# addtt/ladder-vae-pytorch

Measured on NVIDIA B200. Metric: train images/s (CIFAR10 15-layer LVAE), higher is better.
Workload: dtype bf16

## Files before the change

### ladder-vae-pytorch_b200/csrc/wgrad_tcgen05.cu

```cuda
#include "common.cuh"
#include <cuda.h>
#include <string.h>

namespace {

constexpr int WG_THREADS_TC = 192;
constexpr int WG_TILE = 128;
constexpr int WG_BLK_BYTES = WG_TILE * 64 * 2;
constexpr int WG_MAX_PAIRS = 5;
constexpr int WG_PAIR_SLOTS = 4;
constexpr int WG_B_SLOTS = 2;
constexpr int WG_HALO_BYTES = 18 * 16 * 128;
constexpr int WG_HALO_STAGE_BYTES = WG_HALO_BYTES + WG_BLK_BYTES;
constexpr int WG_HALO_STAGES = 3;

struct WgParams {
  int M_total, H, W;
  int n_pairs;
  int n_bblk;
  int tmem_cols;
  int tiles_per_cta;
  int dy_c0;
  int halo, tiles_x, tiles_per_img;
  int in_stride;

  int8_t a_src[2 * WG_MAX_PAIRS], a_dx[2 * WG_MAX_PAIRS], a_dy[2 * WG_MAX_PAIRS];
};

__device__ __forceinline__ uint32_t smem_u32(const void* p) { return (uint32_t)__cvta_generic_to_shared(p); }
__device__ __forceinline__ void mbar_init(uint32_t bar, uint32_t count) {
  asm volatile("mbarrier.init.shared::cta.b64 [%0], %1;" ::"r"(bar), "r"(count));
}
__device__ __forceinline__ void mbar_expect_tx(uint32_t bar, uint32_t bytes) {
  asm volatile("mbarrier.arrive.expect_tx.shared::cta.b64 _, [%0], %1;" ::"r"(bar), "r"(bytes) : "memory");
}
__device__ __forceinline__ uint32_t mbar_try_wait(uint32_t bar, uint32_t parity) {
  uint32_t ok;
  asm volatile(
      "{\n\t.reg .pred p;\n\t"
      "mbarrier.try_wait.parity.shared::cta.b64 p, [%1], %2;\n\t"
      "selp.u32 %0, 1, 0, p;\n\t}"
      : "=r"(ok) : "r"(bar), "r"(parity) : "memory");
  return ok;
}
__device__ __forceinline__ void mbar_wait(uint32_t bar, uint32_t parity) {
  while (!mbar_try_wait(bar, parity)) {}
}
__device__ __forceinline__ void tma_load_4d(uint32_t dst, const CUtensorMap* tm, uint32_t bar, int c0, int c1, int c2, int c3) {
  asm volatile(
      "cp.async.bulk.tensor.4d.shared::cluster.global.mbarrier::complete_tx::bytes [%0], [%1, {%3, %4, %5, %6}], [%2];"
      ::"r"(dst), "l"(tm), "r"(bar), "r"(c0), "r"(c1), "r"(c2), "r"(c3) : "memory");
}
__device__ __forceinline__ uint64_t umma_desc_mn_sw128(uint32_t saddr, uint32_t lbo_bytes, uint32_t sbo_bytes = 1024) {
  uint64_t d = 0;
  d |= (uint64_t)((saddr & 0x3FFFF) >> 4);
  d |= (uint64_t)((lbo_bytes >> 4) & 0x3FFF) << 16;
  d |= (uint64_t)(sbo_bytes >> 4) << 32;
  d |= (uint64_t)1 << 46;
  d |= (uint64_t)2 << 61;
  return d;
}
__device__ __forceinline__ void umma_bf16(uint32_t d_tmem, uint64_t adesc, uint64_t bdesc, uint32_t idesc, uint32_t accumulate) {
  asm volatile(
      "{\n\t.reg .pred p;\n\t"
      "setp.ne.b32 p, %4, 0;\n\t"
      "tcgen05.mma.cta_group::1.kind::f16 [%0], %1, %2, %3, p;\n\t}"
      ::"r"(d_tmem), "l"(adesc), "l"(bdesc), "r"(idesc), "r"(accumulate) : "memory");
}
__device__ __forceinline__ uint32_t elect_one() {
  uint32_t pred = 0;
  asm volatile(
      "{\n\t.reg .pred p;\n\t"
      "elect.sync _|p, 0xffffffff;\n\t"
      "selp.u32 %0, 1, 0, p;\n\t}"
      : "=r"(pred));
  return pred;
}
__device__ __forceinline__ void umma_commit(uint32_t bar) {
  asm volatile("tcgen05.commit.cta_group::1.mbarrier::arrive::one.shared::cluster.b64 [%0];" ::"r"(bar) : "memory");
}
__device__ __forceinline__ void tc_fence_before() { asm volatile("tcgen05.fence::before_thread_sync;" ::: "memory"); }
__device__ __forceinline__ void tc_fence_after() { asm volatile("tcgen05.fence::after_thread_sync;" ::: "memory"); }
__device__ __forceinline__ void tmem_ld32(uint32_t taddr, uint32_t* r) {
  asm volatile(
      "tcgen05.ld.sync.aligned.32x32b.x32.b32 {%0,%1,%2,%3,%4,%5,%6,%7,%8,%9,%10,%11,%12,%13,%14,%15,"
      "%16,%17,%18,%19,%20,%21,%22,%23,%24,%25,%26,%27,%28,%29,%30,%31}, [%32];"
      : "=r"(r[0]), "=r"(r[1]), "=r"(r[2]), "=r"(r[3]), "=r"(r[4]), "=r"(r[5]), "=r"(r[6]), "=r"(r[7]), "=r"(r[8]),
        "=r"(r[9]), "=r"(r[10]), "=r"(r[11]), "=r"(r[12]), "=r"(r[13]), "=r"(r[14]), "=r"(r[15]), "=r"(r[16]),
        "=r"(r[17]), "=r"(r[18]), "=r"(r[19]), "=r"(r[20]), "=r"(r[21]), "=r"(r[22]), "=r"(r[23]), "=r"(r[24]),
        "=r"(r[25]), "=r"(r[26]), "=r"(r[27]), "=r"(r[28]), "=r"(r[29]), "=r"(r[30]), "=r"(r[31])
      : "r"(taddr));
  asm volatile("tcgen05.wait::ld.sync.aligned;" ::: "memory");
}

__global__ void __launch_bounds__(WG_THREADS_TC, 1)
wgrad_tc_kernel(const __grid_constant__ CUtensorMap tmX, const __grid_constant__ CUtensorMap tmX2,
                const __grid_constant__ CUtensorMap tmDY, const __grid_constant__ CUtensorMap tmGp, const WgParams p) {
  extern __shared__ uint8_t smem_raw[];
  uint8_t* smem = smem_raw + ((1024u - (smem_u32(smem_raw) & 1023u)) & 1023u);
  uint8_t* sPair = smem;
  uint8_t* sB = sPair + WG_PAIR_SLOTS * 2 * WG_BLK_BYTES;
  uint8_t* sOnes = p.halo ? smem + WG_HALO_STAGES * WG_HALO_STAGE_BYTES
                          : sB + WG_B_SLOTS * p.n_bblk * WG_BLK_BYTES;
  uint64_t* bars = (uint64_t*)(sOnes + WG_BLK_BYTES);
  uint32_t* tmem_slot = (uint32_t*)(bars + 16);
  const uint32_t bar0 = smem_u32(bars);
  auto BAR = [&](int i) { return bar0 + 8u * (uint32_t)i; };
  const int warp = threadIdx.x >> 5, lane = threadIdx.x & 31;
  const int n_tiles = p.halo ? (p.M_total / (p.H * p.W)) * p.tiles_per_img : (p.M_total + WG_TILE - 1) / WG_TILE;
  const int tile_beg = blockIdx.x * p.tiles_per_cta;
  const int tile_end = min(n_tiles, tile_beg + p.tiles_per_cta);
  const int N = 64 * p.n_bblk;

  if (threadIdx.x == 0) {
    for (int i = 0; i < 13; ++i) mbar_init(BAR(i), 1);
    asm volatile("fence.mbarrier_init.release.cluster;" ::: "memory");
  }
  for (int i = threadIdx.x; i < WG_BLK_BYTES / 4; i += WG_THREADS_TC) ((uint32_t*)sOnes)[i] = 0x3F803F80u;
  asm volatile("fence.proxy.async.shared::cta;" ::: "memory");
  if (warp == 1) {
    asm volatile("tcgen05.alloc.cta_group::1.sync.aligned.shared::cta.b32 [%0], %1;" ::"r"(smem_u32(tmem_slot)), "r"(p.tmem_cols) : "memory");
    asm volatile("tcgen05.relinquish_alloc_permit.cta_group::1.sync.aligned;" ::: "memory");
  }
  tc_fence_before();
  __syncthreads();
  tc_fence_after();
  const uint32_t tmem_base = *tmem_slot;
  pdl_wait();
  pdl_launch();

  if (warp == 0) {
    if (p.halo) {
      int st = 0;
      uint32_t ph = 0;
      for (int tile = tile_beg; tile < tile_end; ++tile) {
        const int n0 = tile / p.tiles_per_img;
        const int r = tile - n0 * p.tiles_per_img;
        const int ty = r / p.tiles_x, tx = r - ty * p.tiles_x;
        mbar_wait(BAR(4 + st), ph ^ 1);
        if (elect_one()) {
          uint8_t* stage = smem + st * WG_HALO_STAGE_BYTES;
          mbar_expect_tx(BAR(st), (uint32_t)WG_HALO_STAGE_BYTES);
          tma_load_4d(smem_u32(stage), &tmX, BAR(st), 0, tx * 8 - 1, ty * 16 - 1, n0);
          tma_load_4d(smem_u32(stage + WG_HALO_BYTES), &tmDY, BAR(st), p.dy_c0, tx * 8, ty * 16, n0);
        }
        __syncwarp();
        if (++st == WG_HALO_STAGES) { st = 0; ph ^= 1; }
      }
    } else {
      const int hw = p.H * p.W;
      int ps = 0, bs = 0;
      uint32_t pph = 0, bph = 0;
      for (int tile = tile_beg; tile < tile_end; ++tile) {
        int p0 = tile * WG_TILE;
        int n0 = p0 / hw;
        int rem = p0 - n0 * hw;
        int h0 = rem / p.W;
        int w0 = rem - h0 * p.W;
        mbar_wait(BAR(10 + bs), bph ^ 1);
        if (elect_one()) {
          mbar_expect_tx(BAR(8 + bs), (uint32_t)(p.n_bblk * WG_BLK_BYTES));
          for (int j = 0; j < p.n_bblk; ++j)
            tma_load_4d(smem_u32(sB + (bs * p.n_bblk + j) * WG_BLK_BYTES), &tmDY, BAR(8 + bs), p.dy_c0 + 64 * j, w0, h0, n0);
        }
        __syncwarp();
        if (++bs == WG_B_SLOTS) { bs = 0; bph ^= 1; }
        for (int pr = 0; pr < p.n_pairs; ++pr) {
          mbar_wait(BAR(4 + ps), pph ^ 1);
          if (elect_one()) {
            int nload = 0;
            for (int h = 0; h < 2; ++h) nload += p.a_src[2 * pr + h] < 2 ? 1 : 0;
            mbar_expect_tx(BAR(ps), (uint32_t)(nload * WG_BLK_BYTES));
            for (int h = 0; h < 2; ++h) {
              int src = p.a_src[2 * pr + h];
              if (src < 2)
                tma_load_4d(smem_u32(sPair + (ps * 2 + h) * WG_BLK_BYTES), src ? &tmX2 : &tmX, BAR(ps), 0,
                            w0 * p.in_stride + p.a_dx[2 * pr + h], h0 * p.in_stride + p.a_dy[2 * pr + h], n0);
            }
          }
          __syncwarp();
          if (++ps == WG_PAIR_SLOTS) { ps = 0; pph ^= 1; }
        }
      }
    }
  } else if (warp == 1) {
    {
      const uint32_t tmem_u = __shfl_sync(0xffffffffu, tmem_base, 0);
      const uint32_t idesc = (1u << 4) | (1u << 7) | (1u << 10) | (1u << 15) | (1u << 16) |
                             ((uint32_t)(N >> 3) << 17) | ((uint32_t)(128 >> 4) << 24);
      int ps = 0, bs = 0;
      uint32_t pph = 0, bph = 0;
      if (p.halo) {
        int st = 0;
        uint32_t ph = 0;
        const uint32_t ones = smem_u32(sOnes);
        for (int tile = tile_beg; tile < tile_end; ++tile) {
          mbar_wait(BAR(st), ph);
          tc_fence_after();
          const uint32_t h_addr = smem_u32(smem + st * WG_HALO_STAGE_BYTES);
          const uint32_t b_addr = h_addr + WG_HALO_BYTES;
          if (elect_one()) {
            for (int pr = 0; pr < p.n_pairs; ++pr) {
              const uint32_t a0 = h_addr + (uint32_t)(((1 + p.a_dy[2 * pr]) * 16 + (1 + p.a_dx[2 * pr])) * 128);
              const bool second_ones = p.a_src[2 * pr + 1] == 2;
              const uint32_t a1 = h_addr + (uint32_t)(((1 + p.a_dy[2 * pr + 1]) * 16 + (1 + p.a_dx[2 * pr + 1])) * 128);
              const uint32_t d_tmem = tmem_u + (uint32_t)(pr * N);
#pragma unroll
              for (int k = 0; k < WG_TILE / 16; ++k) {
                const uint32_t ak = a0 + k * 4096;
                const uint32_t lbo = second_ones ? ones - ak : a1 - a0;
                umma_bf16(d_tmem, umma_desc_mn_sw128(ak, lbo, 2048), umma_desc_mn_sw128(b_addr + k * 2048, WG_BLK_BYTES),
                          idesc, (uint32_t)((tile != tile_beg) || k != 0));
              }
            }
            umma_commit(BAR(4 + st));
          }
          __syncwarp();
          if (++st == WG_HALO_STAGES) { st = 0; ph ^= 1; }
        }
        if (elect_one()) umma_commit(BAR(12));
        __syncwarp();
      } else {
      for (int tile = tile_beg; tile < tile_end; ++tile) {
        mbar_wait(BAR(8 + bs), bph);
        tc_fence_after();
        const uint32_t b_addr = smem_u32(sB + bs * p.n_bblk * WG_BLK_BYTES);
        for (int pr = 0; pr < p.n_pairs; ++pr) {
          mbar_wait(BAR(ps), pph);
          tc_fence_after();
          const uint32_t a_addr = smem_u32(sPair + ps * 2 * WG_BLK_BYTES);
          const uint32_t a2 = p.a_src[2 * pr + 1] == 2 ? smem_u32(sOnes) : a_addr + WG_BLK_BYTES;
          const uint32_t lbo_a = a2 - a_addr;
          const uint32_t d_tmem = tmem_u + (uint32_t)(pr * N);
          if (elect_one()) {
#pragma unroll
            for (int k = 0; k < WG_TILE / 16; ++k) {
              umma_bf16(d_tmem, umma_desc_mn_sw128(a_addr + k * 2048, lbo_a), umma_desc_mn_sw128(b_addr + k * 2048, WG_BLK_BYTES),
                        idesc, (uint32_t)((tile != tile_beg) || k != 0));
            }
            umma_commit(BAR(4 + ps));
          }
          __syncwarp();
          if (++ps == WG_PAIR_SLOTS) { ps = 0; pph ^= 1; }
        }
        if (elect_one()) umma_commit(BAR(10 + bs));
        __syncwarp();
        if (++bs == WG_B_SLOTS) { bs = 0; bph ^= 1; }
      }
      if (elect_one()) umma_commit(BAR(12));
      __syncwarp();
      }
    }
  } else {
    const int quad = warp & 3;
    const int row = quad * 32 + lane;
    const bool leader = threadIdx.x == 64;
    mbar_wait(BAR(12), 0);
    tc_fence_after();
    if (tile_beg < tile_end) {
      int nbuf = 0;
      for (int pr = 0; pr < p.n_pairs; ++pr) {
        const uint32_t taddr = tmem_base + ((uint32_t)(quad * 32) << 16) + (uint32_t)(pr * N);
        for (int c0 = 0; c0 < N; c0 += 32, ++nbuf) {
          uint8_t* stg = smem + (nbuf & 1) * WG_BLK_BYTES;
          uint32_t r[32];
          tmem_ld32(taddr + (uint32_t)c0, r);
          if (leader) asm volatile("cp.async.bulk.wait_group.read 1;" ::: "memory");
          asm volatile("bar.sync 1, 128;" ::: "memory");
#pragma unroll
          for (int q = 0; q < 8; ++q)
            *reinterpret_cast<uint4*>(stg + row * 128 + ((q ^ (row & 7)) << 4)) = make_uint4(r[4 * q], r[4 * q + 1], r[4 * q + 2], r[4 * q + 3]);
          asm volatile("fence.proxy.async.shared::cta;" ::: "memory");
          asm volatile("bar.sync 1, 128;" ::: "memory");
          if (leader) {
            asm volatile("cp.reduce.async.bulk.tensor.2d.global.shared::cta.add.tile.bulk_group [%0, {%2, %3}], [%1];"
                         ::"l"(&tmGp), "r"(smem_u32(stg)), "r"(c0), "r"(pr * 128) : "memory");
            asm volatile("cp.async.bulk.commit_group;" ::: "memory");
          }
        }
      }
      if (leader) asm volatile("cp.async.bulk.wait_group 0;" ::: "memory");
    }
  }
  tc_fence_before();
  __syncthreads();
  if (warp == 1) {
    asm volatile("tcgen05.dealloc.cta_group::1.sync.aligned.b32 %0, %1;" ::"r"(tmem_base), "r"(p.tmem_cols) : "memory");
  }
}

struct UnpackDesc {
  const float* gp; float* dw; float* dbias;
  int n_pairs, N, taps, I_real, N_real, clear;
  int8_t kind[2 * WG_MAX_PAIRS];
  int8_t tap[2 * WG_MAX_PAIRS], ci0_blk[2 * WG_MAX_PAIRS];
  int8_t pad_[2];
};
static_assert(sizeof(UnpackDesc) == 80, "UnpackDesc layout is mirrored by engine.py");

constexpr int UNPACK_CO = 16;

__device__ __forceinline__ void unpack_body(const UnpackDesc& d, float (*tile)[9 * 64 + 1]) {
  const int co0 = blockIdx.x * UNPACK_CO;
  if (co0 >= d.N_real) return;
  const int run = d.I_real * d.taps;
  float* gp = const_cast<float*>(d.gp);
  const int n_items = d.n_pairs * 128 * (UNPACK_CO / 4);
  const bool clear = (d.clear & 1) != 0, overwrite = (d.clear & 2) != 0;
  for (int base = threadIdx.x; base < n_items; base += 4 * blockDim.x) {
    float4 v[4];
#pragma unroll
    for (int u = 0; u < 4; ++u) {
      const int idx = base + u * blockDim.x;
      if (idx < n_items) v[u] = *reinterpret_cast<const float4*>(gp + (size_t)(idx / (UNPACK_CO / 4)) * d.N + co0 + 4 * (idx % (UNPACK_CO / 4)));
    }
#pragma unroll
    for (int u = 0; u < 4; ++u) {
      const int idx = base + u * blockDim.x;
      if (idx >= n_items) break;
      const int i = idx / (UNPACK_CO / 4), part = idx % (UNPACK_CO / 4);
      const int blk = i >> 6, ci = i & 63;
      const int kind = d.kind[blk];
      if (clear) *reinterpret_cast<float4*>(gp + (size_t)i * d.N + co0 + 4 * part) = make_float4(0.f, 0.f, 0.f, 0.f);
      const float vv[4] = {v[u].x, v[u].y, v[u].z, v[u].w};
      if (kind == 0) {
        const int cin = d.ci0_blk[blk] * 64 + ci;
        if (cin < d.I_real) {
          const int o = cin * d.taps + d.tap[blk];
#pragma unroll
          for (int e = 0; e < 4; ++e) tile[4 * part + e][o] = vv[e];
        }
      } else if (kind == 1 && ci == 0 && d.dbias) {
#pragma unroll
        for (int e = 0; e < 4; ++e)
          if (co0 + 4 * part + e < d.N_real) {
            if (overwrite) d.dbias[co0 + 4 * part + e] = vv[e];
            else d.dbias[co0 + 4 * part + e] += vv[e];
          }
      }
    }
  }
  __syncthreads();
  const int nco = min(UNPACK_CO, d.N_real - co0);
  float* dst = d.dw + (size_t)co0 * run;
  const int total = nco * run;
  if (overwrite) {
    for (int o = threadIdx.x; o < total; o += blockDim.x) dst[o] = tile[o / run][o % run];
  } else {
    for (int base = threadIdx.x; base < total; base += 4 * blockDim.x) {
      float old[4];
#pragma unroll
      for (int u = 0; u < 4; ++u) { const int o = base + u * blockDim.x; if (o < total) old[u] = dst[o]; }
#pragma unroll
      for (int u = 0; u < 4; ++u) { const int o = base + u * blockDim.x; if (o < total) dst[o] = old[u] + tile[o / run][o % run]; }
    }
  }
}

__global__ void __launch_bounds__(256) wgrad_unpack_kernel(const UnpackDesc* __restrict__ table) {
  pdl_wait();
  pdl_launch();
  __shared__ UnpackDesc d;
  __shared__ float tile[UNPACK_CO][9 * 64 + 1];
  if (threadIdx.x < sizeof(UnpackDesc) / 4)
    reinterpret_cast<uint32_t*>(&d)[threadIdx.x] = reinterpret_cast<const uint32_t*>(table + blockIdx.y)[threadIdx.x];
  __syncthreads();
  unpack_body(d, tile);
}
__global__ void __launch_bounds__(256) wgrad_unpack_one_kernel(const UnpackDesc dpar) {
  pdl_wait();
  pdl_launch();
  __shared__ UnpackDesc d;
  __shared__ float tile[UNPACK_CO][9 * 64 + 1];
  if (threadIdx.x == 0) d = dpar;
  __syncthreads();
  unpack_body(d, tile);
}

void fill_unpack_desc(UnpackDesc* d, const float* gp, float* dw, float* dbias, int N, int ksize, int inputs, int I_real,
                      int N_real, int clear) {
  memset(d, 0, sizeof(*d));
  const int taps = ksize * ksize;
  int nblk = 0;
  for (int t = 0; t < taps; ++t)
    for (int s = 0; s < inputs && nblk < 2 * WG_MAX_PAIRS - 1; ++s, ++nblk) { d->kind[nblk] = 0; d->tap[nblk] = (int8_t)t; d->ci0_blk[nblk] = (int8_t)s; }
  if (nblk % 2 == 0 && nblk < 2 * WG_MAX_PAIRS - 1) { d->kind[nblk] = 2; ++nblk; }
  d->kind[nblk] = 1; ++nblk;
  d->gp = gp; d->dw = dw; d->dbias = dbias; d->n_pairs = nblk / 2; d->N = N; d->taps = taps;
  d->I_real = I_real > 0 ? I_real : 64 * inputs; d->N_real = N_real > 0 ? N_real : N; d->clear = clear;
}

typedef CUresult (*EncodeTiledFn)(CUtensorMap*, CUtensorMapDataType, cuuint32_t, void*, const cuuint64_t*, const cuuint64_t*,
                                  const cuuint32_t*, const cuuint32_t*, CUtensorMapInterleave, CUtensorMapSwizzle,
                                  CUtensorMapL2promotion, CUtensorMapFloatOOBfill);
EncodeTiledFn wg_get_encode() {
  static EncodeTiledFn fn = nullptr;
  if (!fn) {
    void* ptr = nullptr;
    cudaDriverEntryPointQueryResult q;
    if (cudaGetDriverEntryPoint("cuTensorMapEncodeTiled", &ptr, cudaEnableDefault, &q) == cudaSuccess && q == cudaDriverEntryPointSuccess)
      fn = (EncodeTiledFn)ptr;
  }
  return fn;
}

int make_act_map(EncodeTiledFn enc, CUtensorMap* tm, const void* ptr, int B, int H, int W, int C, int bw, int bh, int bn, int st = 1) {
  cuuint64_t gdim[4] = {(cuuint64_t)C, (cuuint64_t)W, (cuuint64_t)H, (cuuint64_t)B};
  cuuint64_t gstr[3] = {(cuuint64_t)C * 2, (cuuint64_t)W * C * 2, (cuuint64_t)H * W * C * 2};
  cuuint32_t box[4] = {64, (cuuint32_t)(bw * st), (cuuint32_t)(bh * st), (cuuint32_t)bn};
  cuuint32_t estr[4] = {1, (cuuint32_t)st, (cuuint32_t)st, 1};
  return (int)enc(tm, CU_TENSOR_MAP_DATA_TYPE_BFLOAT16, 4, (void*)ptr, gdim, gstr, box, estr, CU_TENSOR_MAP_INTERLEAVE_NONE,
                  CU_TENSOR_MAP_SWIZZLE_128B, CU_TENSOR_MAP_L2_PROMOTION_L2_256B, CU_TENSOR_MAP_FLOAT_OOB_FILL_NONE);
}

}

static bool wgrad_shape_ok(int N, int ksize, int inputs) {
  if (!(N == 64 || N == 128) || !(ksize == 1 || ksize == 3) || inputs < 1 || inputs > 2) return false;
  const int nblk = ksize * ksize * inputs;
  const int n_pairs = (nblk + 1 + (nblk % 2 == 0 ? 1 : 0)) / 2;
  return n_pairs <= WG_MAX_PAIRS && n_pairs * N <= 512;
}

LVAE_API long long lvae_wgrad_tc_packed_size(int N, int ksize, int two_inputs) {
  const int inputs = two_inputs ? 2 : 1;
  if (!wgrad_shape_ok(N, ksize, inputs)) return 0;
  const int nblk = ksize * ksize * inputs;
  return (long long)((nblk + 1 + (nblk % 2 == 0 ? 1 : 0)) / 2) * 128 * N;
}
LVAE_API long long lvae_wgrad_tc_workspace(int B, int H, int W, int N, int ksize, int two_inputs) {
  (void)B; (void)H; (void)W;
  return lvae_wgrad_tc_packed_size(N, ksize, two_inputs);
}

static int wgrad_tc_acc_impl(const void* x, const void* x2, const void* dy, float* gp, int B, int H, int W, int N,
                             int ksize, int dyC, int dy_c0, int in_stride, cudaStream_t stream);

LVAE_API int lvae_conv2d_wgrad_tc_acc(const void* x, const void* x2, const void* dy, float* gp, int B, int H, int W, int N,
                                      int ksize, int dyC, int dy_c0, cudaStream_t stream) {
  return wgrad_tc_acc_impl(x, x2, dy, gp, B, H, W, N, ksize, dyC, dy_c0, 1, stream);
}

LVAE_API int lvae_conv2d_wgrad_tc_s2_acc(const void* xs, const void* c, float* gp, int B, int Hg, int Wg, cudaStream_t stream) {
  return wgrad_tc_acc_impl(xs, nullptr, c, gp, B, Hg, Wg, 64, 3, 64, 0, 2, stream);
}

static int wgrad_tc_acc_impl(const void* x, const void* x2, const void* dy, float* gp, int B, int H, int W, int N,
                             int ksize, int dyC, int dy_c0, int in_stride, cudaStream_t stream) {
  LVAE_REQUIRE(x && dy && gp, "conv2d_wgrad_tc: null pointer");
  LVAE_REQUIRE((N == 64 || N == 128) && (ksize == 1 || ksize == 3), "conv2d_wgrad_tc: N must be 64 or 128, ksize 1 or 3");
  LVAE_REQUIRE((W & (W - 1)) == 0 && (H & (H - 1)) == 0 && W <= 128, "conv2d_wgrad_tc: H and W must be powers of two (W <= 128)");
  EncodeTiledFn enc = wg_get_encode();
  if (!enc) { lvae_set_error("conv2d_wgrad_tc: cuTensorMapEncodeTiled unavailable"); return LVAE_ERR_CUDA; }
  const int inputs = x2 ? 2 : 1, taps = ksize * ksize;
  LVAE_REQUIRE(wgrad_shape_ok(N, ksize, inputs), "conv2d_wgrad_tc: too many operand blocks (3x3 over two inputs is not supported)");
  WgParams p{};
  int nblk = 0;
  for (int t = 0; t < taps; ++t) {
    int oy = t / ksize - ksize / 2, ox = t % ksize - ksize / 2;
    for (int s = 0; s < inputs; ++s, ++nblk) { p.a_src[nblk] = (int8_t)s; p.a_dx[nblk] = (int8_t)ox; p.a_dy[nblk] = (int8_t)oy; }
  }
  if (nblk % 2 == 0) { p.a_src[nblk] = 0; p.a_dx[nblk] = 0; p.a_dy[nblk] = 0; ++nblk; }
  p.a_src[nblk] = 2; ++nblk;
  p.n_pairs = nblk / 2;
  p.n_bblk = N / 64;
  p.tmem_cols = 32;
  while (p.tmem_cols < p.n_pairs * N) p.tmem_cols *= 2;
  p.M_total = B * H * W; p.H = H; p.W = W;
  p.in_stride = in_stride;
  p.halo = (in_stride == 1 && ksize == 3 && !x2 && N == 64 && W % 8 == 0 && H % 16 == 0) ? 1 : 0;
  p.tiles_x = W / 8;
  p.tiles_per_img = (W / 8) * (H / 16);
  const int n_tiles = p.halo ? B * p.tiles_per_img : (p.M_total + WG_TILE - 1) / WG_TILE;
  constexpr int WG_TILES_PER_CTA = 8;
  int grid = (n_tiles + WG_TILES_PER_CTA - 1) / WG_TILES_PER_CTA;
  if (grid > lvae_num_sms()) grid = lvae_num_sms();
  if (grid < 1) grid = 1;
  p.tiles_per_cta = (n_tiles + grid - 1) / grid;
  grid = (n_tiles + p.tiles_per_cta - 1) / p.tiles_per_cta;
  int bw = W;
  int bh = 1;
  while (bh * 2 <= H && bh * 2 * bw <= WG_TILE) bh *= 2;
  int bn = WG_TILE / (bw * bh);
  if (p.halo) { bw = 8; bh = 16; bn = 1; }
  CUtensorMap tmX, tmX2, tmDY, tmGp;
  int r = p.halo ? make_act_map(enc, &tmX, x, B, H, W, 64, 16, 18, 1)
                 : make_act_map(enc, &tmX, x, B, H * in_stride, W * in_stride, 64, bw, bh, bn, in_stride);
  if (!r) r = make_act_map(enc, &tmX2, x2 ? x2 : x, B, H, W, 64, bw, bh, bn);
  if (dyC <= 0) dyC = N;
  LVAE_REQUIRE(dy_c0 % 64 == 0 && dy_c0 + N <= dyC, "conv2d_wgrad_tc: bad dY channel window");
  p.dy_c0 = dy_c0;
  if (!r) r = make_act_map(enc, &tmDY, dy, B, H, W, dyC, bw, bh, bn);
  if (!r) {
    cuuint64_t gdim[2] = {(cuuint64_t)N, (cuuint64_t)p.n_pairs * 128};
    cuuint64_t gstr[1] = {(cuuint64_t)N * 4};
    cuuint32_t box[2] = {32, 128};
    cuuint32_t estr[2] = {1, 1};
    r = (int)enc(&tmGp, CU_TENSOR_MAP_DATA_TYPE_FLOAT32, 2, (void*)gp, gdim, gstr, box, estr, CU_TENSOR_MAP_INTERLEAVE_NONE,
                 CU_TENSOR_MAP_SWIZZLE_128B, CU_TENSOR_MAP_L2_PROMOTION_NONE, CU_TENSOR_MAP_FLOAT_OOB_FILL_NONE);
  }
  if (r) { lvae_set_error("conv2d_wgrad_tc: tensor map encode failed: %d", r); return LVAE_ERR_CUDA; }
  const size_t smem = p.halo ? 1024 + (size_t)WG_HALO_STAGES * WG_HALO_STAGE_BYTES + WG_BLK_BYTES + 256
                             : 1024 + (size_t)WG_PAIR_SLOTS * 2 * WG_BLK_BYTES + (size_t)WG_B_SLOTS * p.n_bblk * WG_BLK_BYTES + WG_BLK_BYTES + 256;
  static bool attr = false;
  if (!attr) {
    cudaError_t e = cudaFuncSetAttribute(wgrad_tc_kernel, cudaFuncAttributeMaxDynamicSharedMemorySize, 227 * 1024);
    if (e != cudaSuccess) { lvae_set_error("conv2d_wgrad_tc: cannot raise dynamic smem: %s", cudaGetErrorString(e)); return LVAE_ERR_CUDA; }
    attr = true;
  }
  lvae_launch(wgrad_tc_kernel, grid, WG_THREADS_TC, smem, stream, tmX, tmX2, tmDY, tmGp, p);
  LVAE_COUNT_LAUNCH();
  LVAE_CHECK_LAUNCH("conv2d_wgrad_tc");
  return LVAE_OK;
}

LVAE_API int lvae_wgrad_unpack_desc_size(void) { return (int)sizeof(UnpackDesc); }
LVAE_API int lvae_wgrad_unpack_desc(void* desc_host, const float* gp, float* dw, float* dbias, int N, int ksize, int two_inputs,
                                    int I_real, int N_real, int clear) {
  LVAE_REQUIRE(desc_host && gp && dw, "wgrad_unpack_desc: null pointer");
  LVAE_REQUIRE(wgrad_shape_ok(N, ksize, two_inputs ? 2 : 1), "wgrad_unpack_desc: unsupported shape");
  fill_unpack_desc((UnpackDesc*)desc_host, gp, dw, dbias, N, ksize, two_inputs ? 2 : 1, I_real, N_real, clear);
  return LVAE_OK;
}
LVAE_API int lvae_wgrad_unpack_batched(const void* desc_dev, int n, int max_n_real, cudaStream_t stream) {
  LVAE_REQUIRE(desc_dev && n > 0 && max_n_real > 0, "wgrad_unpack_batched: bad args");
  lvae_launch(wgrad_unpack_kernel, dim3(cdiv(max_n_real, UNPACK_CO), n), 256, 0, stream, (const UnpackDesc*)desc_dev);
  LVAE_COUNT_LAUNCH();
  LVAE_CHECK_LAUNCH("wgrad_unpack");
  return LVAE_OK;
}

LVAE_API int lvae_conv2d_wgrad_tc_s2(const void* xs, const void* c, float* dw, float* dbias, float* ws, int B, int Hg, int Wg,
                                     cudaStream_t stream) {
  LVAE_REQUIRE(xs && c && dw && ws, "conv2d_wgrad_tc_s2: null pointer");
  const long long n = lvae_wgrad_tc_packed_size(64, 3, 0);
  cudaError_t e = cudaMemsetAsync(ws, 0, (size_t)n * 4, stream);
  if (e != cudaSuccess) { lvae_set_error("conv2d_wgrad_tc_s2: memset failed: %s", cudaGetErrorString(e)); return LVAE_ERR_CUDA; }
  int rc = lvae_conv2d_wgrad_tc_s2_acc(xs, c, ws, B, Hg, Wg, stream);
  if (rc) return rc;
  UnpackDesc d;
  fill_unpack_desc(&d, ws, dw, dbias, 64, 3, 1, 64, 64, 0);
  lvae_launch(wgrad_unpack_one_kernel, dim3(cdiv(d.N_real, UNPACK_CO), 1), 256, 0, stream, d);
  LVAE_COUNT_LAUNCH();
  LVAE_CHECK_LAUNCH("wgrad_unpack");
  return LVAE_OK;
}

LVAE_API int lvae_conv2d_wgrad_tc(const void* x, const void* x2, const void* dy, float* dw, float* dbias, float* ws,
                                  int B, int H, int W, int N, int ksize, int I_real, int N_real, int dyC, int dy_c0,
                                  cudaStream_t stream) {
  LVAE_REQUIRE(x && dy && dw && ws, "conv2d_wgrad_tc: null pointer");
  const long long n = lvae_wgrad_tc_packed_size(N, ksize, x2 != nullptr);
  LVAE_REQUIRE(n > 0, "conv2d_wgrad_tc: unsupported shape");
  cudaError_t e = cudaMemsetAsync(ws, 0, (size_t)n * 4, stream);
  if (e != cudaSuccess) { lvae_set_error("conv2d_wgrad_tc: memset failed: %s", cudaGetErrorString(e)); return LVAE_ERR_CUDA; }
  int rc = lvae_conv2d_wgrad_tc_acc(x, x2, dy, ws, B, H, W, N, ksize, dyC, dy_c0, stream);
  if (rc) return rc;
  UnpackDesc d;
  fill_unpack_desc(&d, ws, dw, dbias, N, ksize, x2 ? 2 : 1, I_real, N_real, 0);
  lvae_launch(wgrad_unpack_one_kernel, dim3(cdiv(d.N_real, UNPACK_CO), 1), 256, 0, stream, d);
  LVAE_COUNT_LAUNCH();
  LVAE_CHECK_LAUNCH("wgrad_unpack");
  return LVAE_OK;
}
```

### profiles/wgrad_tap_pairing_check.py

```python
import itertools
import numpy as np

rng = np.random.default_rng(0)
H, W, CI, CO = 6, 5, 3, 4
X = rng.standard_normal((H, W, CI))
DY = rng.standard_normal((H, W, CO))


def at(T, y, x):
    return T[y, x] if 0 <= y < H and 0 <= x < W else np.zeros(T.shape[2])


def true_tap(t):
    return sum(np.outer(at(X, y + t[0], x + t[1]), DY[y, x]) for y in range(H) for x in range(W))


def quadrant(a, b):
    return sum(np.outer(at(X, y + a[0], x + a[1]), at(DY, y + b[0], x + b[1])) for y in range(H) for x in range(W))


S = [(y, x) for y in (-1, 0, 1) for x in (-1, 0, 1)]
rule_ok = lambda a, b: all(a[i] == 0 or b[i] == 0 for i in (0, 1))
n_valid = 0
for a, b in itertools.product(S, S):
    t = (a[0] - b[0], a[1] - b[1])
    exact = max(abs(t[0]), abs(t[1])) <= 1 and np.allclose(quadrant(a, b), true_tap(t), atol=1e-12)
    assert exact == rule_ok(a, b), (a, b, exact)
    n_valid += exact
print("rule 'per axis a = 0 or b = 0' <=> quadrant equals tap a - b: verified for all 81 shift pairs (%d valid)" % n_valid)

cover = [(((-1, -1), (-1, 0)), ((0, -1), (0, 0))), (((0, -1), (0, 0)), ((-1, 0), (0, 0))), (((0, 1), "ones"), ((-1, 0), (0, 0)))]
got = {}
for apair, bpair in cover:
    for a in apair:
        for b in bpair:
            if a == "ones":
                if b == (0, 0):
                    got["bias"] = sum(DY[y, x] for y in range(H) for x in range(W))
            elif rule_ok(a, b):
                got[(a[0] - b[0], a[1] - b[1])] = quadrant(a, b)
assert set(got) == set(S) | {"bias"}
for t in S:
    assert np.allclose(got[t], true_tap(t), atol=1e-12)
assert np.allclose(got["bias"], DY.sum((0, 1)))
print("three M = 128, N = 128 MMAs per k-step cover the nine taps and the bias: 10 of 12 quadrants used, all equal to the true gradient")
```

Baseline: 18890.

## Pair shifted dY halo with shifted X to cover 3x3 wgrad taps in three MMAs

Result: no change. 19070, median of 6 (+1.0%).

```diff
diff --git a/ladder-vae-pytorch_b200/csrc/wgrad_tcgen05.cu b/ladder-vae-pytorch_b200/csrc/wgrad_tcgen05.cu
--- a/ladder-vae-pytorch_b200/csrc/wgrad_tcgen05.cu
+++ b/ladder-vae-pytorch_b200/csrc/wgrad_tcgen05.cu
@@ -10,21 +10,31 @@
 constexpr int WG_MAX_PAIRS = 5;
 constexpr int WG_PAIR_SLOTS = 4;
 constexpr int WG_B_SLOTS = 2;
-constexpr int WG_HALO_BYTES = 18 * 16 * 128;
-constexpr int WG_HALO_STAGE_BYTES = WG_HALO_BYTES + WG_BLK_BYTES;
-constexpr int WG_HALO_STAGES = 3;
+constexpr int WG_MAX_STAGES = 6;
+constexpr int WG_HALO_ROW = 16 * 128;
+constexpr int WG_ONES_BYTES = 3072;
+constexpr int WG_SMEM_LIMIT = 227 * 1024;
+constexpr int WG_SMEM_FIXED = 1024 + WG_ONES_BYTES + 256;
+
+enum WgMode { WG_PAIR = 0, WG_HALO = 1, WG_SINGLE = 2 };
 
 struct WgParams {
   int M_total, H, W;
+  int mode;
   int n_pairs;
   int n_bblk;
+  int N;
   int tmem_cols;
   int tiles_per_cta;
   int dy_c0;
-  int halo, tiles_x, tiles_per_img;
+  int ring_bytes;
+  int stages, stage_bytes;
+  int th, tn, tiles_x, tiles_per_img;
   int in_stride;
 
   int8_t a_src[2 * WG_MAX_PAIRS], a_dx[2 * WG_MAX_PAIRS], a_dy[2 * WG_MAX_PAIRS];
+  int8_t b_dx[2 * WG_MAX_PAIRS], b_dy[2 * WG_MAX_PAIRS];
+  int8_t gp_blk[WG_MAX_PAIRS][2][2];
 };
 
 __device__ __forceinline__ uint32_t smem_u32(const void* p) { return (uint32_t)__cvta_generic_to_shared(p); }
@@ -100,23 +110,23 @@
   uint8_t* smem = smem_raw + ((1024u - (smem_u32(smem_raw) & 1023u)) & 1023u);
   uint8_t* sPair = smem;
   uint8_t* sB = sPair + WG_PAIR_SLOTS * 2 * WG_BLK_BYTES;
-  uint8_t* sOnes = p.halo ? smem + WG_HALO_STAGES * WG_HALO_STAGE_BYTES
-                          : sB + WG_B_SLOTS * p.n_bblk * WG_BLK_BYTES;
-  uint64_t* bars = (uint64_t*)(sOnes + WG_BLK_BYTES);
+  uint8_t* sOnes = smem + p.ring_bytes;
+  uint64_t* bars = (uint64_t*)(sOnes + WG_ONES_BYTES);
   uint32_t* tmem_slot = (uint32_t*)(bars + 16);
   const uint32_t bar0 = smem_u32(bars);
   auto BAR = [&](int i) { return bar0 + 8u * (uint32_t)i; };
   const int warp = threadIdx.x >> 5, lane = threadIdx.x & 31;
-  const int n_tiles = p.halo ? (p.M_total / (p.H * p.W)) * p.tiles_per_img : (p.M_total + WG_TILE - 1) / WG_TILE;
+  const int n_tiles = p.mode == WG_HALO ? ((p.M_total / (p.H * p.W) + p.tn - 1) / p.tn) * p.tiles_per_img
+                                        : (p.M_total + WG_TILE - 1) / WG_TILE;
   const int tile_beg = blockIdx.x * p.tiles_per_cta;
   const int tile_end = min(n_tiles, tile_beg + p.tiles_per_cta);
-  const int N = 64 * p.n_bblk;
+  const int accN = 64 * p.n_bblk;
 
   if (threadIdx.x == 0) {
     for (int i = 0; i < 13; ++i) mbar_init(BAR(i), 1);
     asm volatile("fence.mbarrier_init.release.cluster;" ::: "memory");
   }
-  for (int i = threadIdx.x; i < WG_BLK_BYTES / 4; i += WG_THREADS_TC) ((uint32_t*)sOnes)[i] = 0x3F803F80u;
+  for (int i = threadIdx.x; i < WG_ONES_BYTES / 4; i += WG_THREADS_TC) ((uint32_t*)sOnes)[i] = 0x3F803F80u;
   asm volatile("fence.proxy.async.shared::cta;" ::: "memory");
   if (warp == 1) {
     asm volatile("tcgen05.alloc.cta_group::1.sync.aligned.shared::cta.b32 [%0], %1;" ::"r"(smem_u32(tmem_slot)), "r"(p.tmem_cols) : "memory");
@@ -130,22 +140,33 @@
   pdl_launch();
 
   if (warp == 0) {
-    if (p.halo) {
+    if (p.mode != WG_PAIR) {
+      const int hw = p.H * p.W;
       int st = 0;
       uint32_t ph = 0;
       for (int tile = tile_beg; tile < tile_end; ++tile) {
-        const int n0 = tile / p.tiles_per_img;
-        const int r = tile - n0 * p.tiles_per_img;
-        const int ty = r / p.tiles_x, tx = r - ty * p.tiles_x;
-        mbar_wait(BAR(4 + st), ph ^ 1);
+        mbar_wait(BAR(WG_MAX_STAGES + st), ph ^ 1);
         if (elect_one()) {
-          uint8_t* stage = smem + st * WG_HALO_STAGE_BYTES;
-          mbar_expect_tx(BAR(st), (uint32_t)WG_HALO_STAGE_BYTES);
-          tma_load_4d(smem_u32(stage), &tmX, BAR(st), 0, tx * 8 - 1, ty * 16 - 1, n0);
-          tma_load_4d(smem_u32(stage + WG_HALO_BYTES), &tmDY, BAR(st), p.dy_c0, tx * 8, ty * 16, n0);
+          const uint32_t stage = smem_u32(smem + st * p.stage_bytes);
+          mbar_expect_tx(BAR(st), (uint32_t)p.stage_bytes);
+          if (p.mode == WG_HALO) {
+            const int n0 = (tile / p.tiles_per_img) * p.tn;
+            const int r = tile % p.tiles_per_img;
+            const int ty = r / p.tiles_x, tx = r - ty * p.tiles_x;
+            tma_load_4d(stage, &tmX, BAR(st), 0, tx * 8 - 1, ty * p.th - 1, n0);
+            tma_load_4d(stage + p.tn * (p.th + 2) * WG_HALO_ROW, &tmDY, BAR(st), p.dy_c0, tx * 8 - 1, ty * p.th - 1, n0);
+          } else {
+            const int p0 = tile * WG_TILE;
+            const int n0 = p0 / hw;
+            const int rem = p0 - n0 * hw;
+            const int h0 = rem / p.W, w0 = rem - h0 * p.W;
+            tma_load_4d(stage, &tmX, BAR(st), 0, w0, h0, n0);
+            for (int j = 0; j < p.n_bblk; ++j)
+              tma_load_4d(stage + (1 + j) * WG_BLK_BYTES, &tmDY, BAR(st), p.dy_c0 + 64 * j, w0, h0, n0);
+          }
         }
         __syncwarp();
-        if (++st == WG_HALO_STAGES) { st = 0; ph ^= 1; }
+        if (++st == p.stages) { st = 0; ph ^= 1; }
       }
     } else {
       const int hw = p.H * p.W;
@@ -187,40 +208,55 @@
     {
       const uint32_t tmem_u = __shfl_sync(0xffffffffu, tmem_base, 0);
       const uint32_t idesc = (1u << 4) | (1u << 7) | (1u << 10) | (1u << 15) | (1u << 16) |
-                             ((uint32_t)(N >> 3) << 17) | ((uint32_t)(128 >> 4) << 24);
-      int ps = 0, bs = 0;
-      uint32_t pph = 0, bph = 0;
-      if (p.halo) {
+                             ((uint32_t)(accN >> 3) << 17) | ((uint32_t)(128 >> 4) << 24);
+      const uint32_t ones = smem_u32(sOnes);
+      if (p.mode != WG_PAIR) {
         int st = 0;
         uint32_t ph = 0;
-        const uint32_t ones = smem_u32(sOnes);
+        const int kh = p.th >> 1;
         for (int tile = tile_beg; tile < tile_end; ++tile) {
           mbar_wait(BAR(st), ph);
           tc_fence_after();
-          const uint32_t h_addr = smem_u32(smem + st * WG_HALO_STAGE_BYTES);
-          const uint32_t b_addr = h_addr + WG_HALO_BYTES;
+          const uint32_t x_addr = smem_u32(smem + st * p.stage_bytes);
           if (elect_one()) {
-            for (int pr = 0; pr < p.n_pairs; ++pr) {
-              const uint32_t a0 = h_addr + (uint32_t)(((1 + p.a_dy[2 * pr]) * 16 + (1 + p.a_dx[2 * pr])) * 128);
-              const bool second_ones = p.a_src[2 * pr + 1] == 2;
-              const uint32_t a1 = h_addr + (uint32_t)(((1 + p.a_dy[2 * pr + 1]) * 16 + (1 + p.a_dx[2 * pr + 1])) * 128);
-              const uint32_t d_tmem = tmem_u + (uint32_t)(pr * N);
+            if (p.mode == WG_HALO) {
+              const uint32_t dy_addr = x_addr + (uint32_t)(p.tn * (p.th + 2) * WG_HALO_ROW);
+              for (int pr = 0; pr < p.n_pairs; ++pr) {
+                const int a0 = ((1 + p.a_dy[2 * pr]) * 16 + (1 + p.a_dx[2 * pr])) * 128;
+                const bool second_ones = p.a_src[2 * pr + 1] == 2;
+                const int a1 = ((1 + p.a_dy[2 * pr + 1]) * 16 + (1 + p.a_dx[2 * pr + 1])) * 128;
+                const int b0 = ((1 + p.b_dy[2 * pr]) * 16 + (1 + p.b_dx[2 * pr])) * 128;
+                const int b1 = ((1 + p.b_dy[2 * pr + 1]) * 16 + (1 + p.b_dx[2 * pr + 1])) * 128;
+                const uint32_t d_tmem = tmem_u + (uint32_t)(pr * accN);
+#pragma unroll
+                for (int k = 0; k < WG_TILE / 16; ++k) {
+                  const int img = k / kh, row2 = (k - img * kh) * 2 * WG_HALO_ROW;
+                  const uint32_t ak = x_addr + (uint32_t)(img * (p.th + 2) * WG_HALO_ROW + row2 + a0);
+                  const uint32_t bk = dy_addr + (uint32_t)(img * (p.th + 1) * WG_HALO_ROW + row2 + b0);
+                  const uint32_t lbo_a = second_ones ? ones - ak : (uint32_t)(a1 - a0);
+                  umma_bf16(d_tmem, umma_desc_mn_sw128(ak, lbo_a, WG_HALO_ROW), umma_desc_mn_sw128(bk, (uint32_t)(b1 - b0), WG_HALO_ROW),
+                            idesc, (uint32_t)((tile != tile_beg) || k != 0));
+                }
+              }
+            } else {
+              const uint32_t b_addr = x_addr + WG_BLK_BYTES;
 #pragma unroll
               for (int k = 0; k < WG_TILE / 16; ++k) {
-                const uint32_t ak = a0 + k * 4096;
-                const uint32_t lbo = second_ones ? ones - ak : a1 - a0;
-                umma_bf16(d_tmem, umma_desc_mn_sw128(ak, lbo, 2048), umma_desc_mn_sw128(b_addr + k * 2048, WG_BLK_BYTES),
+                const uint32_t ak = x_addr + k * 2048;
+                umma_bf16(tmem_u, umma_desc_mn_sw128(ak, ones - ak), umma_desc_mn_sw128(b_addr + k * 2048, WG_BLK_BYTES),
                           idesc, (uint32_t)((tile != tile_beg) || k != 0));
               }
             }
-            umma_commit(BAR(4 + st));
+            umma_commit(BAR(WG_MAX_STAGES + st));
           }
           __syncwarp();
-          if (++st == WG_HALO_STAGES) { st = 0; ph ^= 1; }
+          if (++st == p.stages) { st = 0; ph ^= 1; }
         }
         if (elect_one()) umma_commit(BAR(12));
         __syncwarp();
       } else {
+      int ps = 0, bs = 0;
+      uint32_t pph = 0, bph = 0;
       for (int tile = tile_beg; tile < tile_end; ++tile) {
         mbar_wait(BAR(8 + bs), bph);
         tc_fence_after();
@@ -229,13 +265,14 @@
           mbar_wait(BAR(ps), pph);
           tc_fence_after();
           const uint32_t a_addr = smem_u32(sPair + ps * 2 * WG_BLK_BYTES);
-          const uint32_t a2 = p.a_src[2 * pr + 1] == 2 ? smem_u32(sOnes) : a_addr + WG_BLK_BYTES;
-          const uint32_t lbo_a = a2 - a_addr;
-          const uint32_t d_tmem = tmem_u + (uint32_t)(pr * N);
+          const bool second_ones = p.a_src[2 * pr + 1] == 2;
+          const uint32_t d_tmem = tmem_u + (uint32_t)(pr * accN);
           if (elect_one()) {
 #pragma unroll
             for (int k = 0; k < WG_TILE / 16; ++k) {
-              umma_bf16(d_tmem, umma_desc_mn_sw128(a_addr + k * 2048, lbo_a), umma_desc_mn_sw128(b_addr + k * 2048, WG_BLK_BYTES),
+              const uint32_t ak = a_addr + k * 2048;
+              const uint32_t lbo_a = second_ones ? ones - ak : WG_BLK_BYTES;
+              umma_bf16(d_tmem, umma_desc_mn_sw128(ak, lbo_a), umma_desc_mn_sw128(b_addr + k * 2048, WG_BLK_BYTES),
                         idesc, (uint32_t)((tile != tile_beg) || k != 0));
             }
             umma_commit(BAR(4 + ps));
@@ -254,29 +291,34 @@
   } else {
     const int quad = warp & 3;
     const int row = quad * 32 + lane;
-    const bool leader = threadIdx.x == 64;
+    const int half = quad >> 1;
+    const bool leader = lane == 0 && (quad & 1) == 0;
     mbar_wait(BAR(12), 0);
     tc_fence_after();
     if (tile_beg < tile_end) {
       int nbuf = 0;
       for (int pr = 0; pr < p.n_pairs; ++pr) {
-        const uint32_t taddr = tmem_base + ((uint32_t)(quad * 32) << 16) + (uint32_t)(pr * N);
-        for (int c0 = 0; c0 < N; c0 += 32, ++nbuf) {
+        const uint32_t taddr = tmem_base + ((uint32_t)(quad * 32) << 16) + (uint32_t)(pr * accN);
+        for (int c0 = 0; c0 < accN; c0 += 32) {
+          const int j = c0 / p.N;
+          const int blk = p.gp_blk[pr][j][half];
+          if (blk < 0) continue;
           uint8_t* stg = smem + (nbuf & 1) * WG_BLK_BYTES;
           uint32_t r[32];
           tmem_ld32(taddr + (uint32_t)c0, r);
           if (leader) asm volatile("cp.async.bulk.wait_group.read 1;" ::: "memory");
-          asm volatile("bar.sync 1, 128;" ::: "memory");
+          asm volatile("bar.sync %0, 64;" ::"r"(1 + half) : "memory");
 #pragma unroll
           for (int q = 0; q < 8; ++q)
             *reinterpret_cast<uint4*>(stg + row * 128 + ((q ^ (row & 7)) << 4)) = make_uint4(r[4 * q], r[4 * q + 1], r[4 * q + 2], r[4 * q + 3]);
           asm volatile("fence.proxy.async.shared::cta;" ::: "memory");
-          asm volatile("bar.sync 1, 128;" ::: "memory");
+          asm volatile("bar.sync %0, 64;" ::"r"(1 + half) : "memory");
           if (leader) {
             asm volatile("cp.reduce.async.bulk.tensor.2d.global.shared::cta.add.tile.bulk_group [%0, {%2, %3}], [%1];"
-                         ::"l"(&tmGp), "r"(smem_u32(stg)), "r"(c0), "r"(pr * 128) : "memory");
+                         ::"l"(&tmGp), "r"(smem_u32(stg + half * 64 * 128)), "r"(c0 - j * p.N), "r"(blk * 64) : "memory");
             asm volatile("cp.async.bulk.commit_group;" ::: "memory");
           }
+          ++nbuf;
         }
       }
       if (leader) asm volatile("cp.async.bulk.wait_group 0;" ::: "memory");
@@ -464,14 +506,51 @@
   p.a_src[nblk] = 2; ++nblk;
   p.n_pairs = nblk / 2;
   p.n_bblk = N / 64;
-  p.tmem_cols = 32;
-  while (p.tmem_cols < p.n_pairs * N) p.tmem_cols *= 2;
+  p.N = N;
+  for (int pr = 0; pr < p.n_pairs; ++pr)
+    for (int h = 0; h < 2; ++h) { p.gp_blk[pr][0][h] = (int8_t)(2 * pr + h); p.gp_blk[pr][1][h] = -1; }
   p.M_total = B * H * W; p.H = H; p.W = W;
   p.in_stride = in_stride;
-  p.halo = (in_stride == 1 && ksize == 3 && !x2 && N == 64 && W % 8 == 0 && H % 16 == 0) ? 1 : 0;
-  p.tiles_x = W / 8;
-  p.tiles_per_img = (W / 8) * (H / 16);
-  const int n_tiles = p.halo ? B * p.tiles_per_img : (p.M_total + WG_TILE - 1) / WG_TILE;
+  const bool halo = in_stride == 1 && ksize == 3 && !x2 && N == 64 && W % 8 == 0 && H % 8 == 0;
+  p.mode = halo ? WG_HALO : (in_stride == 1 && p.n_pairs == 1) ? WG_SINGLE : WG_PAIR;
+  if (halo) {
+    static const int8_t A[6][2] = {{-1, -1}, {-1, 0}, {0, -1}, {0, 0}, {0, 1}, {0, 0}};
+    static const int8_t Bs[6][2] = {{0, -1}, {0, 0}, {-1, 0}, {0, 0}, {-1, 0}, {0, 0}};
+    p.n_pairs = 3;
+    p.n_bblk = 2;
+    for (int i = 0; i < 6; ++i) {
+      p.a_src[i] = i == 5 ? 2 : 0;
+      p.a_dy[i] = A[i][0]; p.a_dx[i] = A[i][1];
+      p.b_dy[i] = Bs[i][0]; p.b_dx[i] = Bs[i][1];
+    }
+    for (int m = 0; m < 3; ++m)
+      for (int j = 0; j < 2; ++j)
+        for (int h = 0; h < 2; ++h) {
+          const int ia = 2 * m + h, ib = 2 * m + j;
+          const int ay = A[ia][0], ax = A[ia][1], by = Bs[ib][0], bx = Bs[ib][1];
+          int blk = -1;
+          if (p.a_src[ia] == 2) blk = (by == 0 && bx == 0) ? 9 : -1;
+          else if ((ay == 0 || by == 0) && (ax == 0 || bx == 0)) blk = (ay - by + 1) * 3 + (ax - bx + 1);
+          p.gp_blk[m][j][h] = (int8_t)blk;
+        }
+    p.th = H % 16 == 0 ? 16 : 8;
+    p.tn = 16 / p.th;
+    p.tiles_x = W / 8;
+    p.tiles_per_img = (W / 8) * (H / p.th);
+    p.stage_bytes = p.tn * (2 * p.th + 3) * WG_HALO_ROW;
+  } else if (p.mode == WG_SINGLE) {
+    p.stage_bytes = WG_BLK_BYTES * (1 + p.n_bblk);
+  }
+  if (p.mode == WG_PAIR) {
+    p.ring_bytes = WG_PAIR_SLOTS * 2 * WG_BLK_BYTES + WG_B_SLOTS * p.n_bblk * WG_BLK_BYTES;
+  } else {
+    p.stages = (WG_SMEM_LIMIT - WG_SMEM_FIXED) / p.stage_bytes;
+    if (p.stages > WG_MAX_STAGES) p.stages = WG_MAX_STAGES;
+    p.ring_bytes = p.stages * p.stage_bytes;
+  }
+  p.tmem_cols = 32;
+  while (p.tmem_cols < p.n_pairs * 64 * p.n_bblk) p.tmem_cols *= 2;
+  const int n_tiles = halo ? (B + p.tn - 1) / p.tn * p.tiles_per_img : (p.M_total + WG_TILE - 1) / WG_TILE;
   constexpr int WG_TILES_PER_CTA = 8;
   int grid = (n_tiles + WG_TILES_PER_CTA - 1) / WG_TILES_PER_CTA;
   if (grid > lvae_num_sms()) grid = lvae_num_sms();
@@ -482,29 +561,28 @@
   int bh = 1;
   while (bh * 2 <= H && bh * 2 * bw <= WG_TILE) bh *= 2;
   int bn = WG_TILE / (bw * bh);
-  if (p.halo) { bw = 8; bh = 16; bn = 1; }
   CUtensorMap tmX, tmX2, tmDY, tmGp;
-  int r = p.halo ? make_act_map(enc, &tmX, x, B, H, W, 64, 16, 18, 1)
-                 : make_act_map(enc, &tmX, x, B, H * in_stride, W * in_stride, 64, bw, bh, bn, in_stride);
+  int r = halo ? make_act_map(enc, &tmX, x, B, H, W, 64, 16, p.th + 2, p.tn)
+               : make_act_map(enc, &tmX, x, B, H * in_stride, W * in_stride, 64, bw, bh, bn, in_stride);
   if (!r) r = make_act_map(enc, &tmX2, x2 ? x2 : x, B, H, W, 64, bw, bh, bn);
   if (dyC <= 0) dyC = N;
   LVAE_REQUIRE(dy_c0 % 64 == 0 && dy_c0 + N <= dyC, "conv2d_wgrad_tc: bad dY channel window");
   p.dy_c0 = dy_c0;
-  if (!r) r = make_act_map(enc, &tmDY, dy, B, H, W, dyC, bw, bh, bn);
+  if (!r) r = halo ? make_act_map(enc, &tmDY, dy, B, H, W, dyC, 16, p.th + 1, p.tn)
+                   : make_act_map(enc, &tmDY, dy, B, H, W, dyC, bw, bh, bn);
   if (!r) {
-    cuuint64_t gdim[2] = {(cuuint64_t)N, (cuuint64_t)p.n_pairs * 128};
+    cuuint64_t gdim[2] = {(cuuint64_t)N, (cuuint64_t)lvae_wgrad_tc_packed_size(N, ksize, x2 != nullptr) / N};
     cuuint64_t gstr[1] = {(cuuint64_t)N * 4};
-    cuuint32_t box[2] = {32, 128};
+    cuuint32_t box[2] = {32, 64};
     cuuint32_t estr[2] = {1, 1};
     r = (int)enc(&tmGp, CU_TENSOR_MAP_DATA_TYPE_FLOAT32, 2, (void*)gp, gdim, gstr, box, estr, CU_TENSOR_MAP_INTERLEAVE_NONE,
                  CU_TENSOR_MAP_SWIZZLE_128B, CU_TENSOR_MAP_L2_PROMOTION_NONE, CU_TENSOR_MAP_FLOAT_OOB_FILL_NONE);
   }
   if (r) { lvae_set_error("conv2d_wgrad_tc: tensor map encode failed: %d", r); return LVAE_ERR_CUDA; }
-  const size_t smem = p.halo ? 1024 + (size_t)WG_HALO_STAGES * WG_HALO_STAGE_BYTES + WG_BLK_BYTES + 256
-                             : 1024 + (size_t)WG_PAIR_SLOTS * 2 * WG_BLK_BYTES + (size_t)WG_B_SLOTS * p.n_bblk * WG_BLK_BYTES + WG_BLK_BYTES + 256;
+  const size_t smem = (size_t)WG_SMEM_FIXED + p.ring_bytes;
   static bool attr = false;
   if (!attr) {
-    cudaError_t e = cudaFuncSetAttribute(wgrad_tc_kernel, cudaFuncAttributeMaxDynamicSharedMemorySize, 227 * 1024);
+    cudaError_t e = cudaFuncSetAttribute(wgrad_tc_kernel, cudaFuncAttributeMaxDynamicSharedMemorySize, WG_SMEM_LIMIT);
     if (e != cudaSuccess) { lvae_set_error("conv2d_wgrad_tc: cannot raise dynamic smem: %s", cudaGetErrorString(e)); return LVAE_ERR_CUDA; }
     attr = true;
   }
diff --git a/profiles/wgrad_tap_pairing_check.py b/profiles/wgrad_tap_pairing_check.py
--- a/profiles/wgrad_tap_pairing_check.py
+++ b/profiles/wgrad_tap_pairing_check.py
@@ -44,3 +44,81 @@
     assert np.allclose(got[t], true_tap(t), atol=1e-12)
 assert np.allclose(got["bias"], DY.sum((0, 1)))
 print("three M = 128, N = 128 MMAs per k-step cover the nine taps and the bias: 10 of 12 quadrants used, all equal to the true gradient")
+
+ROW, HROW = 128, 16 * 128
+A_SH = [(-1, -1), (-1, 0), (0, -1), (0, 0), (0, 1), "ones"]
+B_SH = [(0, -1), (0, 0), (-1, 0), (0, 0), (-1, 0), (0, 0)]
+
+
+def gp_blk(m, j, h):
+    a, b = A_SH[2 * m + h], B_SH[2 * m + j]
+    if a == "ones":
+        return 9 if b == (0, 0) else -1
+    return (a[0] - b[0] + 1) * 3 + (a[1] - b[1] + 1) if rule_ok(a, b) else -1
+
+
+def halo_path(Xb, DYb):
+    Bn, Hh, Ww, ci = Xb.shape
+    co = DYb.shape[3]
+    th = 16 if Hh % 16 == 0 else 8
+    tn, kh = 16 // th, th // 2
+    x_bytes, stage_bytes = tn * (th + 2) * HROW, tn * (2 * th + 3) * HROW
+    ones = stage_bytes
+    smem = np.zeros(((stage_bytes + 3072) // ROW, 64))
+    smem[ones // ROW:, :] = 1.0
+    D = np.zeros((3, 128, 128))
+    for n0 in range(0, Bn, tn):
+        for ty in range(Hh // th):
+            for tx in range(Ww // 8):
+                smem[:stage_bytes // ROW] = 0.0
+                for i in range(tn):
+                    for r in range(th + 2):
+                        for c in range(16):
+                            y, x, n = ty * th - 1 + r, tx * 8 - 1 + c, n0 + i
+                            if n < Bn and 0 <= y < Hh and 0 <= x < Ww:
+                                smem[(i * (th + 2) * HROW + r * HROW + c * ROW) // ROW, :ci] = Xb[n, y, x]
+                                if r < th + 1:
+                                    smem[(x_bytes + i * (th + 1) * HROW + r * HROW + c * ROW) // ROW, :co] = DYb[n, y, x]
+                for m in range(3):
+                    off = lambda s: ((1 + s[0]) * 16 + (1 + s[1])) * ROW
+                    a0, b0, b1 = off(A_SH[2 * m]), off(B_SH[2 * m]), off(B_SH[2 * m + 1])
+                    for k in range(8):
+                        img, row2 = k // kh, (k % kh) * 2 * HROW
+                        ak = img * (th + 2) * HROW + row2 + a0
+                        bk = x_bytes + img * (th + 1) * HROW + row2 + b0
+                        lbo_a = ones - ak if A_SH[2 * m + 1] == "ones" else off(A_SH[2 * m + 1]) - a0
+                        lbo_b = b1 - b0
+                        assert lbo_a > 0 and lbo_b > 0 and lbo_a % 16 == 0
+                        for kk in range(16):
+                            kr = (kk // 8) * 2048 + (kk % 8) * ROW
+                            Am = np.concatenate([smem[(ak + h * lbo_a + kr) // ROW] for h in range(2)])
+                            Bm = np.concatenate([smem[(bk + j * lbo_b + kr) // ROW] for j in range(2)])
+                            assert (ak + lbo_a + kr) // ROW < len(smem)
+                            D[m] += np.outer(Am, Bm)
+    Gp = np.zeros((10, 64, 64))
+    seen = []
+    for m in range(3):
+        for j in range(2):
+            for h in range(2):
+                blk = gp_blk(m, j, h)
+                if blk >= 0:
+                    Gp[blk] += D[m, 64 * h:64 * h + 64, 64 * j:64 * j + 64]
+                    seen.append(blk)
+    assert sorted(seen) == list(range(10)), seen
+    return Gp
+
+
+for Bn, Hh, Ww in ((3, 8, 8), (1, 16, 16), (2, 16, 8), (1, 32, 16)):
+    ci_, co_ = 5, 7
+    Xb = rng.standard_normal((Bn, Hh, Ww, ci_))
+    DYb = rng.standard_normal((Bn, Hh, Ww, co_))
+    Gp = halo_path(Xb, DYb)
+    Xp = np.pad(Xb, ((0, 0), (1, 1), (1, 1), (0, 0)))
+    for t in range(9):
+        oy, ox = t // 3 - 1, t % 3 - 1
+        ref = np.einsum("nyxc,nyxo->co", Xp[:, 1 + oy:1 + oy + Hh, 1 + ox:1 + ox + Ww], DYb)
+        assert np.allclose(Gp[t, :ci_, :co_], ref, atol=1e-9), (Bn, Hh, Ww, t)
+    assert np.allclose(Gp[9, :, :co_], DYb.sum((0, 1, 2))[None, :], atol=1e-9)
+    assert not Gp[:9, ci_:, :].any() and not Gp[:, :, co_:].any()
+print("halo path addressing (16-pixel halo pitch, zero fill, odd batch at 8x8, ones tile above the ring): packed gradient "
+      "equals the true 3x3 weight and bias gradient")
```
